# CMUAbstract/VINSat

Measured on AMD Instinct MI355X. Metric: BA iterations/sec (500 poses, 50k landmarks) + final pose RMSE vs ref, higher is better.
Workload: dtype f64; 1 GPU; C3: 500-pose / 50000-observation window, 20-call schedule (10 landmark-only + 10 full); poses=500, observations=50000, windows_per_gpu=1, parallelism=replicas1, devices_visible=1, ranks_per_device=1

## Files before the change

__graft_entry__.py:

```python
import os
import subprocess
import sys

ROOT = os.path.dirname(os.path.abspath(__file__))
if ROOT not in sys.path:
    sys.path.insert(0, ROOT)


def build():
    subprocess.check_call(["make", "-C", os.path.join(ROOT, "vinsat_amd", "csrc"), "-j4"])
    subprocess.call(["make", "-C", os.path.join(ROOT, "tests", "fake_rccl")], stdout=subprocess.DEVNULL, stderr=subprocess.DEVNULL)
    from vinsat_amd import _lib
    lib = _lib.load()
    assert lib.vba_version() >= 100
    import vinsat_amd.ba
    import vinsat_amd.od_pipe


def smoke():
    import numpy as np
    from oracle import ba_oracle as O
    from vinsat_amd import od_pipe, synth
    from vinsat_amd.engine import BAEngine

    lib_path = os.path.join(ROOT, "vinsat_amd", "libvinsat_ba.so")
    if not os.path.exists(lib_path):
        build()
    det, orb = synth.make_sequence("C1")
    win = od_pipe.prepare_window(det, orb)
    st = od_pipe.initial_guess(win)
    n, m = st.shape[0], win.ii.shape[0]
    eng = BAEngine(n, m)
    eng.upload_observations(win.landmarks_xyz, win.landmarks_uv, win.confidences, win.ii, n)
    eng.upload_window(win.intrinsics, win.cumrot_last, win.time_idx)
    lam = 1e-4
    ref, lam_ref = st.copy(), lam
    for it, init in ((0, True), (1, True), (10, False), (11, False)):
        st, lam, hess, ntr, flags = eng.iterate(it, init, lam, st)
        ref, lam_ref, hess_ref, ntr_ref = O.ba_iteration(it, ref, win.cumrot_last, win.landmarks_uv, win.landmarks_xyz,
                                                         win.ii, win.time_idx, win.intrinsics, win.confidences, lam_ref,
                                                         initialize=init)
        err = np.abs(st - ref).max() / np.abs(ref).max()
        assert ntr == ntr_ref and lam == lam_ref, (ntr, ntr_ref, lam, lam_ref)
        assert err < 1e-8, err
    eng.close()
    win2 = od_pipe.prepare_window(*synth.make_two_pass_sequence())
    st2 = win2.states_gt.copy()
    st2[:, :3] += 0.5
    n2, m2 = st2.shape[0], win2.ii.shape[0]
    eng2 = BAEngine(n2, m2)
    eng2.upload_observations(win2.landmarks_xyz, win2.landmarks_uv, win2.confidences, win2.ii, n2)
    eng2.upload_window(win2.intrinsics, win2.cumrot_last, win2.time_idx)
    out2, lam2, _, ntr2, _ = eng2.iterate(12, False, 1e-3, st2)
    ref2, lam_ref2, _, ntr_ref2 = O.ba_iteration(12, st2, win2.cumrot_last, win2.landmarks_uv, win2.landmarks_xyz, win2.ii, win2.time_idx,
                                                win2.intrinsics, win2.confidences, 1e-3, initialize=False)
    err2 = np.abs(out2 - ref2).max() / np.abs(ref2).max()
    assert ntr2 == ntr_ref2 and lam2 == lam_ref2 and err2 < 1e-8, (ntr2, ntr_ref2, lam2, lam_ref2, err2)
    eng2.close()
    print(f"smoke ok: 4 BA calls on cuda:0, max rel state error vs oracle {err:.2e}; a call across gaps of 935 / 510 s {err2:.2e}")


if __name__ == "__main__":
    build()
    if len(sys.argv) > 1 and sys.argv[1] == "smoke":
        smoke()
```

vinsat_amd/csrc/vba_obs.hip:

```cpp
#include "vba_decide.h"
#include <cstdlib>
#include "vba_device.h"
#include "vba_dyn_body.h"
#include "vba_launch.h"
#include "vba_step.h"

namespace vba {

__device__ __forceinline__ void begin_call_scalars(WinScalars& sc, int par, bool keep_wmax = false) {
    sc.done = 0;
    sc.n_trials = 0;
    sc.fl[par] = 0u;
    if (!keep_wmax) sc.wmax_bits[par] = 0ull;
    sc.sum_abs_rpred = 0.0;
}

template <bool HIST0>
__global__ __launch_bounds__(kObsBlock) void k_obs_residual(DevView V, double* abs_out ) {
    __shared__ double red[kObsBlock / 64];
    __shared__ unsigned lh[HIST0 ? 1024 : 1];
    const int w = blockIdx.y;
    VBA_SKIP_CALL(V, w);
    const int m = V.m[w];
    const size_t ob = (size_t)w * V.obs_stride;
// ... 199 lines not shown
    if (blockIdx.x == 0 && threadIdx.x == 0) front_commit(V, w, hit, bin_out, rank_out, in_bin_out, inline_select);
    return hit ? kWarmHit : kWarmMiss;
}

template <int ITEMS>
__global__ __launch_bounds__(256) void k_select_warm(DevView V) {
    __shared__ unsigned lds_u[260];
    __shared__ double red[5][4];
    const int w = blockIdx.y;
    WinScalars& sc = V.sc[w];
    const int t = threadIdx.x;
    const bool fold_here = V.call >= 0 && V.fold && sc.pending == V.call - 1 && sc.call_idx == V.call - 1;
    if (!fold_here) VBA_SKIP_CALL(V, w);
    const double* keys = V.absr + 2 * (size_t)w * V.m_max;
    const int64_t count = 2 * (int64_t)V.m[w];
    if ((int64_t)blockIdx.x * 256 * ITEMS >= count) return;
    constexpr bool PRELOAD = ITEMS <= 8;
    constexpr int PAIRS = ITEMS / 2;
    const double2* keys2 = reinterpret_cast<const double2*>(keys);
    const int64_t npair = count / 2;
    double2 pk[PAIRS];
#pragma unroll
    for (int it = 0; it < PAIRS; ++it) {
        const int64_t idx = ((int64_t)blockIdx.x * PAIRS + it) * 256 + t;
        pk[it] = idx < npair ? keys2[idx] : make_double2(0.0, 0.0);
    }
    const unsigned long long lo = sc.warm_lo[V.par];
    unsigned bin, in_bin;
    long long rank;
    if (warm_front(V, w, fold_here, false, 2 * V.m_max, red, lds_u, bin, rank, in_bin) != kWarmHit) return;
    if constexpr (!PRELOAD) {
        double2 (&kk)[PAIRS] = pk;
        unsigned long long mbits = 0ull;
#pragma unroll
        for (int it = 0; it < PAIRS; ++it) {
            const int64_t idx = ((int64_t)blockIdx.x * PAIRS + it) * 256 + t;
            const bool have = idx < npair;
            if (have && warm_bin(f64_bits(kk[it].x), lo, V.warm_shift) == bin) mbits |= 1ull << (2 * it);
            if (have && warm_bin(f64_bits(kk[it].y), lo, V.warm_shift) == bin) mbits |= 2ull << (2 * it);
        }
        const unsigned mine = (unsigned)__popcll(mbits);
        const unsigned inc = wave_inclusive_scan_u32(mine);
        __syncthreads();
        if ((t & 63) == 63) lds_u[t >> 6] = inc;
        __syncthreads();
        if (t == 0) {
            const unsigned total = lds_u[0] + lds_u[1] + lds_u[2] + lds_u[3];
            lds_u[4] = total ? atomicAdd(&sc.sel_cnt, total) : 0u;
        }
        __syncthreads();
        unsigned at = lds_u[4] + inc - mine;
        for (int q = 0; q < (t >> 6); ++q) at += lds_u[q];
        double* list = V.ckeys + 2 * (size_t)w * V.m_max;
#pragma unroll
        for (int it = 0; it < PAIRS; ++it) {
            if (mbits & (1ull << (2 * it))) list[at++] = kk[it].x;
            if (mbits & (2ull << (2 * it))) list[at++] = kk[it].y;
        }
        return;
    }
    auto take = [&](unsigned long long key, bool have) {
        const bool match = have && warm_bin(key, lo, V.warm_shift) == bin;
        const unsigned long long mask = __ballot(match);
        if (mask) {
            const int lane = t & 63;
            const int leader = __ffsll((long long)mask) - 1;
            unsigned base = 0;
            if (lane == leader) base = atomicAdd(&sc.sel_cnt, (unsigned)__popcll(mask));
            base = (unsigned)__builtin_amdgcn_readlane((int)base, leader);
            if (match) V.ckeys[2 * (size_t)w * V.m_max + base + (unsigned)__popcll(mask & ((1ull << lane) - 1ull))] = bits_f64(key);
        }
    };
    if constexpr (PRELOAD) {
#pragma unroll 8
        for (int it = 0; it < PAIRS; ++it) {
            const int64_t idx = ((int64_t)blockIdx.x * PAIRS + it) * 256 + t;
            const bool have = idx < npair;
            take(f64_bits(pk[it].x), have);
            take(f64_bits(pk[it].y), have);
        }
    }
}

__device__ __forceinline__ double select_finish_list(const DevView& V, int w, const double* ck, int64_t cap, unsigned cnt, long long want,
                                                     int mode, unsigned long long warm_base, bool speculate, unsigned* lh ,
                                                     unsigned* lds_u , unsigned long long* skeys ) {
    const WinScalars& sc = V.sc[w];
    unsigned long long pre[4];
    if (V.sel_nslots > 0 && ck == V.sel_slots) {
        unsigned lo_q = 0;
#pragma unroll
        for (int j = 0; j < 4; ++j) pre[j] = 0ull;
        for (int r = 0; r < V.sel_nslots; ++r) {
            const double* slot = ck + (size_t)r * V.sel_slot_stride;
            const unsigned c_r = (unsigned)slot[0];
#pragma unroll
            for (int j = 0; j < 4; ++j) {
                const unsigned q = threadIdx.x + 256u * j;
                if (q >= lo_q && q < lo_q + c_r && q < cnt) pre[j] = f64_bits(slot[1 + (q - lo_q)]);
            }
            lo_q += c_r;
        }
    } else {
#pragma unroll
        for (int j = 0; j < 4; ++j) {
            const unsigned q = threadIdx.x + 256u * j;
            pre[j] = ((int64_t)q < cap && (speculate || q < cnt)) ? f64_bits(ck[q]) : 0ull;
        }
    }
    if (mode == 1 && cnt <= 1024u && V.warm_shift >= 8) {
        const int t = threadIdx.x;
        const int sh = V.warm_shift - 8;
        lh[t] = 0u;
        if (t == 0) { lds_u[16] = 0u; lds_u[17] = 0u; lds_u[18] = 0u; }
        __syncthreads();
        unsigned sb4[4];
#pragma unroll
        for (int j = 0; j < 4; ++j) {
            const unsigned q = t + 256u * j;
            sb4[j] = (unsigned)((pre[j] - warm_base) >> sh) & 255u;
            if (q < cnt) atomicAdd(&lh[sb4[j]], 1u);
        }
        __syncthreads();
        const unsigned c = lh[t];
        const unsigned inc = wave_inclusive_scan_u32(c);
        if ((t & 63) == 63) lds_u[t >> 6] = inc;
        __syncthreads();
        unsigned base = 0;
        for (int q = 0; q < (t >> 6); ++q) base += lds_u[q];
        const long long excl = (long long)base + inc - c;
        if (want >= excl && want < excl + (long long)c) { lds_u[16] = (unsigned)t; lds_u[17] = (unsigned)(want - excl); }
        __syncthreads();
        const unsigned tb = lds_u[16], r = lds_u[17];
#pragma unroll
        for (int j = 0; j < 4; ++j) {
            const unsigned q = t + 256u * j;
            if (q < cnt && sb4[j] == tb) {
                const unsigned slot = atomicAdd(&lds_u[18], 1u);
                skeys[slot] = pre[j];
            }
        }
        __syncthreads();
        const unsigned k = lds_u[18];
        for (unsigned q = t; q < k; q += 256) {
            const unsigned long long key = skeys[q];
            unsigned below = 0;
            for (unsigned j = 0; j < k; ++j) {
                const unsigned long long o = skeys[j];
                below += (o < key) || (o == key && j < q);
            }
            if (below == r) skeys[1024] = key;
        }
        __syncthreads();
        return bits_f64(skeys[1024]);
    }
    if (cnt <= (mode ? (unsigned)kWarmCount : 1024u)) {
#pragma unroll
        for (int j = 0; j < 4; ++j) {
            const unsigned q = threadIdx.x + 256u * j;
            if (q < cnt) skeys[q] = pre[j];
        }
        __syncthreads();
        for (unsigned q = threadIdx.x; q < cnt; q += 256) {
            const unsigned long long key = skeys[q];
            long long below = 0;
            for (unsigned j = 0; j < cnt; ++j) {
                const unsigned long long o = skeys[j];
                below += (o < key) || (o == key && j < q);
            }
            if (below == want) skeys[1024] = key;
        }
        __syncthreads();
        return bits_f64(skeys[1024]);
    }
    if (mode == 1) {
        unsigned long long prefix = 0ull;
        long long rank = want;
        int remaining = V.warm_shift;
        if (remaining > 11) {
            remaining -= 11;
            for (int b = threadIdx.x; b < kSelBins; b += 256) lh[b] = 0u;
            if (threadIdx.x == 0) lds_u[18] = 0u;
            __syncthreads();
            for (unsigned q = threadIdx.x; q < cnt; q += 256) {
                const unsigned long long rel = f64_bits(ck[q]) - warm_base;
                atomicAdd(&lh[(unsigned)(rel >> remaining) & 2047u], 1u);
            }
            __syncthreads();
            unsigned sub_cnt;
            {
                unsigned loc[8];
                select_load(lh, kSelBins, loc);
// ... 165 lines not shown
            DecideOut d;
            if (!fold_decide(V, w, dec_red, d)) return;
        }
        dynamics_block(V, w, blockIdx.x - nb_acc);
        return;
    }
    const int n = V.n[w];
    if (blockIdx.x * PPB >= n) return;
    VBA_ASTAMP(0);
    const StepParams& prm = V.prm;
    const int sub = threadIdx.x % G;
    const size_t ob = (size_t)w * V.obs_stride;
    const size_t mb = (size_t)w * V.m_max;
    double wmax_l = 0.0;
    const int gstride = BATCH ? (int)gridDim.x : 0;
    int pf_beg = 0, pf_end = 0;
    if (BATCH) {
        const int i0 = blockIdx.x * PPB + threadIdx.x / G;
        if (i0 < n) {
            const int* ptr0 = V.pose_ptr + 2 * ob;
            pf_beg = ptr0[i0];
            pf_end = ptr0[i0 + 1];
        }
    }
    for (int grp = blockIdx.x; grp * PPB < n; grp += gstride) {
    const int i = grp * PPB + threadIdx.x / G;
    const size_t pb = (size_t)w * V.n_max + (i < n ? i : 0);

    struct Obs { double x, y, z, u, v, c; };
    struct alignas(8) D2 { double a, b; };
    struct Obs2 { D2 x, y, z, u, v, c; };
    auto load = [&](int k) {
        Obs o;
        o.x = V.ox[ob + k]; o.y = V.oy[ob + k]; o.z = V.oz[ob + k];
        o.u = V.ou[ob + k]; o.v = V.ov[ob + k]; o.c = V.oconf[ob + k];
        return o;
    };
    auto load2 = [&](int k) {
        Obs2 o;
        o.x = *reinterpret_cast<const D2*>(V.ox + ob + k); o.y = *reinterpret_cast<const D2*>(V.oy + ob + k);
        o.z = *reinterpret_cast<const D2*>(V.oz + ob + k); o.u = *reinterpret_cast<const D2*>(V.ou + ob + k);
        o.v = *reinterpret_cast<const D2*>(V.ov + ob + k); o.c = *reinterpret_cast<const D2*>(V.oconf + ob + k);
        return o;
    };

    unsigned hloc[8] = {};
    if (V.sel_inline && !ordered) select_load(hist0_of(V, w, V.par), kSelBins, hloc);
    PoseCam pc{};
    int beg = 0, end = 0;
    Obs ring[kAccDepth]{};
    Obs2 nxt{}, nxt2{};
#ifndef VBA_ACC_PAIR_DEPTH
#define VBA_ACC_PAIR_DEPTH 1
#endif
    constexpr bool kPairDepth2 = BATCH && PAIR && VBA_ACC_PAIR_DEPTH == 2;
    if (i < n) {
        pose_camera(V.states + pb * 10, V.intr + pb * 4, pc);
        if (BATCH) {
            beg = pf_beg;
            end = pf_end;
        } else {
            beg = early_beg;
            end = early_end;
        }
        if (PAIR) {
            if (beg + 2 * sub < end) nxt = load2(beg + 2 * sub);
            if (kPairDepth2 && beg + 2 * sub + 2 * G < end) nxt2 = load2(beg + 2 * sub + 2 * G);
        } else {
#pragma unroll
            for (int d = 0; d < kAccDepth; ++d)
                if (beg + sub + d * G < end) ring[d] = load(beg + sub + d * G);
        }
    }
    if (BATCH) {
        const int in = i + gstride * PPB;
        pf_beg = pf_end = 0;
        if (in < n) {
            const int* ptr = V.pose_ptr + 2 * ob;
            pf_beg = ptr[in];
            pf_end = ptr[in + 1];
        }
    }

    VBA_ASTAMP(1);
    RobustParams rp;
    if (BATCH) {
        rp.c = sc.c_obs;
    } else if (V.sel_inline) {
        unsigned bin, in_bin;
        long long rank;
        if (ordered) {
            if (warm_front(V, w, fold_here, true, V.bucket_cap, dec_red, sel_u, bin, rank, in_bin) != kWarmHit) return;
        } else {
            if (!front_resolve(V, w, hloc, V.bucket_cap, sel_u, bin, rank, in_bin)) return;
        }
        const unsigned long long lo = sc.warm_lo[V.par];
        const double* bucket = V.wbucket + (((size_t)w * 2 + V.par) * kSelBins + bin) * (size_t)V.bucket_cap;
        rp.c = select_finish_list(V, w, bucket, V.bucket_cap, in_bin, rank, 1, lo + ((unsigned long long)(bin - 1u) << V.warm_shift), false,
                                  sel_lh, sel_u, sel_keys);
        if (ordered && blockIdx.x == 0 && threadIdx.x == 0) sc.c_obs = rp.c;
    } else if (V.median_ready) {
        rp.c = sc.c_obs;
    } else {
        rp.c = select_finish(V, w, sel_lh, sel_u, sel_keys);
        if (blockIdx.x == 0) {
            if (threadIdx.x == 0) sc.c_obs = rp.c;
            unsigned* h0 = hist0_of(V, w, V.par);
            for (int b = threadIdx.x; b < kSelBins; b += 256) h0[b] = 0u;
        }
    }
    VBA_ASTAMP(2);
    rp.inv_c = 1.0 / rp.c;
    rp.inv_c2 = 1.0 / (rp.c * rp.c);
    rp.am2 = prm.am2;
    rp.inv_am2 = 1.0 / prm.am2;
    rp.expo = prm.expo;
    rp.alpha_is_2 = prm.alpha_is_2;
    rp.expo_is_mhalf = prm.expo == -0.5;

    constexpr bool CAM = G <= 16 || F32;
    double acc[32];
#pragma unroll
    for (int q = 0; q < 32; ++q) acc[q] = 0.0;
    double cM[5] = {0, 0, 0, 0, 0}, cT[9] = {0, 0, 0, 0, 0, 0, 0, 0, 0}, cS[3] = {0, 0, 0};
    if (i < n) {
        auto process = [&](double ox_, double oy_, double oz_, double ou_, double ov_, double oc_, int k) {
            double u, v, cam[3], d;
            project(pc, ox_, oy_, oz_, u, v, cam, d);
            const double ru = ou_ - u, rv = ov_ - v;
            const double wr = robust_weight_raw(rp, ru, rv);
            V.wraw[mb + k] = wr;
            wmax_l = fmax(wmax_l, wr);
            const double wc = wr * oc_;
            auto cam_sums = [&](double a00, double a02, double a11, double a12, double g0, double g1, double g2, double h0, double h1,
                                double h2) {
                const double w00 = wc * a00, w02 = wc * a02, w11 = wc * a11, w12 = wc * a12;
                cM[0] = fma(w00, a00, cM[0]); cM[1] = fma(w00, a02, cM[1]);
                cM[2] = fma(w11, a11, cM[2]); cM[3] = fma(w11, a12, cM[3]);
                cM[4] = fma(w02, a02, fma(w12, a12, cM[4]));
                cT[0] = fma(w00, g0, cT[0]); cT[1] = fma(w00, g1, cT[1]); cT[2] = fma(w00, g2, cT[2]);
                cT[3] = fma(w11, h0, cT[3]); cT[4] = fma(w11, h1, cT[4]); cT[5] = fma(w11, h2, cT[5]);
                cT[6] = fma(w02, g0, fma(w12, h0, cT[6])); cT[7] = fma(w02, g1, fma(w12, h1, cT[7]));
                cT[8] = fma(w02, g2, fma(w12, h2, cT[8]));
                const double wg0 = wc * g0, wg1 = wc * g1, wg2 = wc * g2, wh0 = wc * h0, wh1 = wc * h1, wh2 = wc * h2;
                acc[15] = fma(wg0, g0, fma(wh0, h0, acc[15])); acc[16] = fma(wg0, g1, fma(wh0, h1, acc[16]));
                acc[17] = fma(wg0, g2, fma(wh0, h2, acc[17])); acc[18] = fma(wg1, g1, fma(wh1, h1, acc[18]));
                acc[19] = fma(wg1, g2, fma(wh1, h2, acc[19])); acc[20] = fma(wg2, g2, fma(wh2, h2, acc[20]));
                cS[0] = fma(w00, ru, cS[0]); cS[1] = fma(w11, rv, cS[1]); cS[2] = fma(w02, ru, fma(w12, rv, cS[2]));
                acc[24] = fma(wg0, ru, fma(wh0, rv, acc[24])); acc[25] = fma(wg1, ru, fma(wh1, rv, acc[25]));
                acc[26] = fma(wg2, ru, fma(wh2, rv, acc[26]));
            };
            if constexpr (F32) {
                const CamJac32 j = cam_jacobian_f32(pc, cam, d);
                cam_sums(j.a00, j.a02, j.a11, j.a12, j.g0, j.g1, j.g2, j.h0, j.h1, j.h2);
            } else if (CAM) {
                const double live = cam[2] > kZMin ? 1.0 : 0.0;
                const double a00 = pc.fx * d, a11 = pc.fy * d;
                const double dl = d * live;
                const double a02 = -(a00 * (cam[0] * dl)), a12 = -(a11 * (cam[1] * dl));
                const double x = cam[0], y = cam[1], z = cam[2];
                const double b00 = 2.0 * a00, b02 = 2.0 * a02, b11 = 2.0 * a11, b12 = 2.0 * a12;
                const double g0 = -(b02 * y), g1 = fma(b02, x, -(b00 * z)), g2 = b00 * y;
                const double h0 = fma(b11, z, -(b12 * y)), h1 = b12 * x, h2 = -(b11 * x);
                cam_sums(a00, a02, a11, a12, g0, g1, g2, h0, h1, h2);
            } else {
                double J[12];
                project_jacobian(pc, cam, d, J);
                int q = 0;
#pragma unroll
                for (int a = 0; a < 6; ++a) {
                    const double ja = wc * J[a], jb = wc * J[6 + a];
#pragma unroll
                    for (int b = a; b < 6; ++b) { acc[q] = fma(ja, J[b], fma(jb, J[6 + b], acc[q])); ++q; }
                    acc[21 + a] = fma(ja, ru, fma(jb, rv, acc[21 + a]));
                }
            }
        };
        if (PAIR) {
            int k = beg + 2 * sub;
            while (k < end) {
                const int kn = k + 2 * G;
                const Obs2 cur = nxt;
                if (kPairDepth2) {
                    nxt = nxt2;
                    if (kn + 2 * G < end) nxt2 = load2(kn + 2 * G);
                } else if (kn < end) nxt = load2(kn);
                process(cur.x.a, cur.y.a, cur.z.a, cur.u.a, cur.v.a, cur.c.a, k);
                if (k + 1 < end) process(cur.x.b, cur.y.b, cur.z.b, cur.u.b, cur.v.b, cur.c.b, k + 1);
                k = kn;
            }
        } else {
            int k = beg + sub;
            while (k < end) {
                const int kn = k + G;
                const Obs cur = ring[0];
#pragma unroll
                for (int d = 0; d + 1 < kAccDepth; ++d) ring[d] = ring[d + 1];
                if (k + kAccDepth * G < end) ring[kAccDepth - 1] = load(k + kAccDepth * G);
                process(cur.x, cur.y, cur.z, cur.u, cur.v, cur.c, k);
                k = kn;
            }
        }
    }
    VBA_ASTAMP(3);
    if (CAM) {
        const double* R = pc.R;
        const double M[3][3] = {{cM[0], 0.0, cM[1]}, {0.0, cM[2], cM[3]}, {cM[1], cM[3], cM[4]}};
        double Y[3][3];
#pragma unroll
        for (int a = 0; a < 3; ++a)
#pragma unroll
            for (int kk = 0; kk < 3; ++kk) Y[a][kk] = fma(R[3 * a], M[0][kk], fma(R[3 * a + 1], M[1][kk], R[3 * a + 2] * M[2][kk]));
#pragma unroll
        for (int a = 0; a < 3; ++a) {
#pragma unroll
            for (int b = a; b < 3; ++b)
                acc[sym6(a, b)] = fma(Y[a][0], R[3 * b], fma(Y[a][1], R[3 * b + 1], Y[a][2] * R[3 * b + 2]));
#pragma unroll
            for (int c = 0; c < 3; ++c)
                acc[sym6(a, 3 + c)] = -fma(R[3 * a], cT[c], fma(R[3 * a + 1], cT[3 + c], R[3 * a + 2] * cT[6 + c]));
            acc[21 + a] = -fma(R[3 * a], cS[0], fma(R[3 * a + 1], cS[1], R[3 * a + 2] * cS[2]));
        }
    }
    VBA_ASTAMP(4);
    int own = 0;
    halving_steps<G, 32, 1>(acc, sub, own);
    if (G == 64) acc[0] += shfl_xor_f64_c<32>(acc[0]);
    if (i < n && sub < 32) {
        double* H = V.Hraw + pb * 21;
        double* B = V.braw + pb * 6;
        constexpr int kOwn = 32 / (G < 32 ? G : 32);
#pragma unroll
        for (int j = 0; j < kOwn; ++j) {
            const int q = own + j;
            if (q < 21) H[q] = acc[j];
            else if (q < 27) B[q - 21] = acc[j];
        }
    }
    VBA_ASTAMP(5);
    if (!BATCH) break;
    }
    wmax_l = wave_max(wmax_l);
    if ((threadIdx.x & 63) == 0) wmx[threadIdx.x >> 6] = wmax_l;
    __syncthreads();
    if (threadIdx.x == 0) {
        const double mx = fmax(fmax(wmx[0], wmx[1]), fmax(wmx[2], wmx[3]));
        atomicMax(V.wmax_ext ? V.wmax_ext : &sc.wmax_bits[V.par], f64_bits(mx));
    }
    VBA_ASTAMP(6);
}

constexpr int kEdgesPerBlock16 = 15;

template <int EMIT, int FUSED, int PART = 0, int TILES = 1>
__global__ __launch_bounds__(kObsBlock) void k_trial(DevView V) {
    static_assert(PART == 0 || FUSED == 0, "split launches exist for the plain geometry only");
    static_assert(TILES == 1 || (PART == 0 && FUSED == 0), "tiled observation blocks exist for the plain one-grid geometry only");
    constexpr bool FORM = FUSED == 1 || FUSED == 2;
    __shared__ double red[kObsBlock / 64];
    __shared__ double redt[TILES > 1 ? 2 * TILES * (kObsBlock / 64) : 1];
    __shared__ unsigned lh[EMIT == 2 ? kSelBins : (EMIT == 1 ? 1024 : 1)];
    __shared__ double snew[FORM ? (kObsBlock + 1) * 10 : 1];
    __shared__ int lpose[FORM ? kObsBlock : 1];
    __shared__ unsigned wlead[FORM ? 4 : 1];
    const int w = blockIdx.y;
    int early_pose = 0, early_prev = 0;
    constexpr bool kEarlyPose = FUSED == 1 || FUSED == 2;
    if (kEarlyPose && PART != 2) {
        const int64_t ke = min((int64_t)blockIdx.x * kObsBlock + threadIdx.x, V.m_max - 1);
        const int* op = V.opose + 2 * (size_t)w * V.obs_stride;
        early_pose = op[ke];
        early_prev = op[ke > 0 ? ke - 1 : 0];
    }
    VBA_SKIP_CALL(V, w);
    WinScalars& sc = V.sc[w];
// ... 559 lines not shown
```

vinsat_amd/csrc/vba_solve_cr.hip:

```cpp
#include "vba_solve_cr_body.h"

namespace vba {

#ifdef VBA_RESIDENT_STAMPS
VBA_KSTAMP_FETCH(fetch_kstamps_cr)
#endif

template <bool PIVOT>
__global__ __launch_bounds__(256) void k_cr_level01(DevView V, int s) {
    __shared__ __attribute__((aligned(16))) double blk[7 * 252];
    cr_level01_body<PIVOT>(V, s, blockIdx.y, blockIdx.x, blk);
}

template <bool PIVOT>
static void launch_cr_level01_t(const DevView& V, int n0_max, hipStream_t s) {
    hipLaunchKernelGGL(k_cr_level01<PIVOT>, dim3((n0_max + 3) / 4, V.W), dim3(256), 0, s, V, V.chunk);
}
template <bool PIVOT, int PRE>
static void launch_reduced_cr_t(const DevView& V, size_t lds, hipStream_t s) {
    hipLaunchKernelGGL((k_solve_reduced_cr<PIVOT, PRE>), dim3(V.W), dim3(kCrThreads), lds, s, V, V.chunk);
}

static int n0_max_of(const DevView& V) { return (V.n_max + V.chunk - 1) / V.chunk - 1; }
static int n0_min_of(const DevView& V) { return (V.n_min + V.chunk - 1) / V.chunk - 1; }

void launch_cr_tail2(const DevView& V, bool pivot, hipStream_t s) {
    const size_t lds = cr_tail2_lds_bytes(n0_max_of(V));
    if (pivot) launch_reduced_cr_t<true, 2>(V, lds, s);
    else launch_reduced_cr_t<false, 2>(V, lds, s);
}

void launch_cr_front2(const DevView& V, bool pivot, hipStream_t s) {
    const int n0_max = n0_max_of(V);
    if (n0_max < kCrSplitMin) return;
    if (pivot) launch_cr_level01_t<true>(V, n0_max, s);
    else launch_cr_level01_t<false>(V, n0_max, s);
    launch_cr_tail2(V, pivot, s);
}

void launch_cr_short(const DevView& V, bool pivot, hipStream_t s) {
    const int n0_max = n0_max_of(V);
    if (n0_min_of(V) >= kCrSplitMin || n0_max <= 0) return;
    const int nb = n0_max < kCrSplitMin ? n0_max : kCrSplitMin - 1;
    const size_t lds = (size_t)nb * 252 * sizeof(double);
    if (pivot) launch_reduced_cr_t<true, 0>(V, lds, s);
    else launch_reduced_cr_t<false, 0>(V, lds, s);
}

void launch_solve_cr(const DevView& V, bool pivot, hipStream_t s) {
    launch_cr_front2(V, pivot, s);
    launch_cr_short(V, pivot, s);
}

hipError_t configure_cr_device() {
    const LdsLimit set[] = {
        {reinterpret_cast<const void*>(k_solve_reduced_cr<false, 0>), kCrLdsCap}, {reinterpret_cast<const void*>(k_solve_reduced_cr<true, 0>), kCrLdsCap},
        {reinterpret_cast<const void*>(k_solve_reduced_cr<false, 2>), kCrTail2LdsCap}, {reinterpret_cast<const void*>(k_solve_reduced_cr<true, 2>), kCrTail2LdsCap}};
    return set_lds_limits(set);
}

}
```

vinsat_amd/csrc/vba_solve_cr_body.h:

```cpp
#pragma once

#include "vba_solve_step.h"
#include "vba_solve_units.h"

namespace vba {


struct CrLanes {
    int grp, own, ownst;
    int lr, lk;
    int offA[5], offB0[5], offB1[5];
    bool hiB[5];
};

__device__ __forceinline__ CrLanes cr_lanes(int lane) {
    CrLanes g;
    g.grp = lane < 9 ? 0 : (lane < 18 ? 1 : (lane < 27 ? 2 : (lane == 27 ? 3 : 4)));
    const int c = g.grp < 3 ? lane - 9 * g.grp : 0;
    g.own = g.grp == 0 ? 81 + c : (g.grp == 1 ? c : (g.grp == 2 ? 162 + c : 243));
    g.ownst = g.grp == 3 ? 1 : 9;
    g.lr = lane & 15;
    g.lk = lane >> 4;
#pragma unroll
    for (int st = 0; st < 5; ++st) {
// ... 139 lines not shown
        const double* l = cL + (size_t)(in ? q : 0) * 171;
        const double* r_ = cR + (size_t)(in ? q : 0) * 171;
#pragma unroll
        for (int it = 0; it < 2; ++it) {
            const int r = it ? r1 : r0, cc = it ? c1 : c0;
            const bool ok = in && lane + 64 * it < 81;
            lv[u][it] = ok ? l[r * 19 + 1 + cc] : 0.0;
            lw[u][it] = ok ? l[r * 19 + 10 + cc] : 0.0;
            rv[u][it] = ok ? r_[r * 19 + 1 + cc] : 0.0;
            rw[u][it] = ok ? r_[r * 19 + 10 + cc] : 0.0;
            dv[u][it] = ok ? bands[j * 243 + 81 + lane + 64 * it] : 0.0;
        }
        gv[u] = (in && lane < 9) ? rhs[j * 9 + lane] - l[lane * 19] - r_[lane * 19] : 0.0;
    }
    between();
#pragma unroll
    for (int u = 0; u < NB; ++u) {
        const int q = q0 + u * stride;
        if (q >= 0 && q < n1) {
            double* B = dst + (size_t)u * dst_stride * 252;
#pragma unroll
            for (int it = 0; it < 2; ++it) {
                const int i = lane + 64 * it;
                if (i < 81) {
                    const int r = it ? r1 : r0, cc = it ? c1 : c0;
                    B[i] = q == 0 ? 0.0 : -lv[u][it];
                    B[81 + i] = dv[u][it] - lw[u][it] - rv[u][it] + (r == cc ? lam32 : 0.0);
                    B[162 + i] = q == n1 - 1 ? 0.0 : -rw[u][it];
                }
            }
            if (lane < 9) B[243 + lane] = gv[u];
        }
    }
}

template <bool PIVOT>
__device__ __forceinline__ void cr_level01_body(const DevView& V, int s, int w, int t, double* blk) {
    VBA_SKIP_CALL(V, w);
    WinScalars& sc = V.sc[w];
    if (sc.done || !solver_mine<PIVOT>(V, sc)) return;
    const int n1 = n_separators(V.n[w], s);
    if (n1 < kCrSplitMin || n1 > 4 * kCrMax || 4 * t >= n1) return;
    const int lane = threadIdx.x & 63, wv = threadIdx.x >> 6;
    const size_t rb = (size_t)w * V.p_max;
    const double lam32 = (double)(float)sc.lam[V.par];
    const int q0 = 4 * t;
    CrLanes g;
    cr_fill<2>(V, w, s, n1, lam32, q0 + wv, 4, blk + (size_t)wv * 252, 4, lane, [&]() { g = cr_lanes(lane); });
    __syncthreads();
    bool bad = false;
    auto store_P = [&](int u) {
        double* P = V.csol2 + (rb + q0 + u) * 171;
        const double* B = blk + (size_t)u * 252;
        for (int e = lane; e < 171; e += 64) P[e] = e < 81 ? B[e] : B[81 + e];
    };
    if (q0 + 2 * wv < n1) cr_eliminate<PIVOT>(blk + (size_t)(2 * wv) * 252, g, lane, bad);
    __syncthreads();
    if (wv < 3) {
        const int u = 2 * wv + 1;
        if (q0 + u < n1) cr_fold(blk + (size_t)u * 252, blk + (size_t)(u - 1) * 252, blk + (size_t)(u + 1) * 252, q0 + u + 1 < n1, g);
    } else {
        store_P(0);
        if (q0 + 2 < n1) store_P(2);
    }
    __syncthreads();
    if (wv < 2) {
        const int u = 4 * wv + 1;
        if (q0 + u < n1) cr_eliminate<PIVOT>(blk + (size_t)u * 252, g, lane, bad);
    }
    __syncthreads();
    if (wv == 0) {
        if (q0 + 3 < n1) {
            cr_fold(blk + 3 * 252, blk + 1 * 252, blk + 5 * 252, q0 + 5 < n1, g);
            wave_sync_lds();
            double* R = V.cL2 + rb * 171 + (size_t)t * 252;
            for (int e = lane; e < 252; e += 64) R[e] = blk[3 * 252 + e];
        }
    } else if (wv == 1) {
        if (q0 + 1 < n1) store_P(1);
    }
    report_pivot<PIVOT>(bad, sc, lane, V.par);
}

template <bool PIVOT, int PRE, int kCrThreads>
__device__ __forceinline__ void reduced_cr_body(const DevView& V, int s, int w, double* smem) {
    VBA_SKIP_CALL(V, w);
    int tsi = 0;
    const bool tson = threadIdx.x == 0;
    VBA_KSTAMP(tson, tsi++);
    WinScalars& sc = V.sc[w];
    if (sc.done || !solver_mine<PIVOT>(V, sc)) return;
    const int n0 = n_separators(V.n[w], s);
    if (n0 <= 0) return;
    if (PRE ? (n0 < kCrSplitMin || n0 > (PRE == 3 ? 8 : (PRE == 2 ? 4 : 2)) * kCrMax) : (n0 >= kCrSplitMin || n0 > kCrMax)) return;
    const int n1 = PRE == 3 ? n0 / 8 : (PRE == 2 ? n0 / 4 : (PRE ? n0 / 2 : n0));
    const int tid = threadIdx.x, lane = tid & 63, wave = tid >> 6;
    constexpr int NW = kCrThreads / 64;
    const size_t rb = (size_t)w * V.p_max;
    const double lam32 = (double)(float)sc.lam[V.par];
    CrLanes g;
    if (PRE) {
        const double* R = V.cL2 + rb * 171;
        constexpr int kFill = (kCrMax * 252 + kCrThreads - 1) / kCrThreads;
        double v[kFill];
#pragma unroll
        for (int k = 0; k < kFill; ++k) {
            const int idx = tid + k * kCrThreads;
            v[k] = idx < n1 * 252 ? R[idx] : 0.0;
        }
        g = cr_lanes(lane);
#pragma unroll
        for (int k = 0; k < kFill; ++k) {
            const int idx = tid + k * kCrThreads;
            if (idx < n1 * 252) smem[idx] = v[k];
        }
    } else {
        cr_fill<kCrMax / NW>(V, w, s, n1, lam32, wave, NW, smem + (size_t)wave * 252, NW, lane, [&]() { g = cr_lanes(lane); });
    }
    __syncthreads();
    VBA_KSTAMP(tson, tsi++);
    bool bad = false;
    int h = 1, lv = 0;
    for (;; h <<= 1, ++lv) {
        const int cnt = n1 >> lv;
        const int nel = (cnt + 1) / 2;
#pragma nounroll
        for (int t = wave; t < nel; t += NW)
            cr_eliminate<PIVOT>(smem + (size_t)((2 * t + 1) * h - 1) * 252, g, lane, bad);
        __syncthreads();
        VBA_KSTAMP(tson, tsi++);
        if (cnt <= 1) break;
        const int nk = cnt / 2;
#pragma nounroll
        for (int t = wave; t < nk; t += NW) {
            const int j = (2 * t + 2) * h - 1;
            const bool has_p = j + h < n1;
            cr_fold(smem + (size_t)j * 252, smem + (size_t)(j - h) * 252, smem + (size_t)(has_p ? j + h : j) * 252, has_p, g);
        }
        VBA_KSTAMP(tson, 64 + tsi);
        __syncthreads();
        VBA_KSTAMP(tson, tsi++);
    }
    for (; h >= 1; h >>= 1, --lv) {
        const int cnt = n1 >> lv;
        const int nel = (cnt + 1) / 2;
        for (int idx = tid; idx < nel * 9; idx += kCrThreads) {
            const int t = idx / 9, r = idx % 9;
            const int k = (2 * t + 1) * h - 1;
            double* B = smem + (size_t)k * 252;
            double x = B[243 + r];
            if (k - h >= 0) {
                const double* xm = smem + (size_t)(k - h) * 252 + 243;
#pragma unroll
                for (int q = 0; q < 9; ++q) x -= B[r * 9 + q] * xm[q];
            }
            if (k + h < n1) {
                const double* xp = smem + (size_t)(k + h) * 252 + 243;
#pragma unroll
                for (int q = 0; q < 9; ++q) x -= B[162 + r * 9 + q] * xp[q];
            }
            B[243 + r] = x;
        }
        __syncthreads();
        VBA_KSTAMP(tson, tsi++);
    }
    if (PRE == 3) {
        double* x2 = smem + (size_t)n1 * 252;
        double* x1 = x2 + (size_t)((n0 + 7) / 8) * 9;
        auto x_odd = [&](int q) -> const double* {
            return (q & 7) == 7 ? smem + (size_t)(q >> 3) * 252 + 243 : ((q & 7) == 3 ? x2 + (size_t)(q >> 3) * 9 : x1 + (size_t)(q >> 2) * 9);
        };
        auto solve_from = [&](int q, int r, int h) {
            const double* P = V.csol2 + (rb + q) * 171;
            double x = P[162 + r];
            if (q - h >= 0) {
                const double* xm = x_odd(q - h);
#pragma unroll
                for (int k = 0; k < 9; ++k) x -= P[r * 9 + k] * xm[k];
            }
            if (q + h < n0) {
                const double* xp = x_odd(q + h);
#pragma unroll
                for (int k = 0; k < 9; ++k) x -= P[81 + r * 9 + k] * xp[k];
            }
            return x;
        };
        for (int idx = tid; idx < ((n0 + 7) / 8) * 9; idx += kCrThreads) {
            const int q = 8 * (idx / 9) + 3, r = idx % 9;
            if (q < n0) x2[(size_t)(q >> 3) * 9 + r] = solve_from(q, r, 4);
        }
        __syncthreads();
        for (int idx = tid; idx < ((n0 + 3) / 4) * 9; idx += kCrThreads) {
            const int q = 4 * (idx / 9) + 1, r = idx % 9;
            if (q < n0) x1[(size_t)(q >> 2) * 9 + r] = solve_from(q, r, 2);
        }
        __syncthreads();
        for (int idx = tid; idx < n0 * 9; idx += kCrThreads) {
            const int q = idx / 9, r = idx % 9;
            V.rx[rb * 9 + idx] = (q & 1) ? x_odd(q)[r] : solve_from(q, r, 1);
        }
    } else if (PRE == 2) {
        double* x1 = smem + (size_t)n1 * 252;
        auto x_odd = [&](int q) -> const double* {
            return (q & 3) == 3 ? smem + (size_t)(q >> 2) * 252 + 243 : x1 + (size_t)(q >> 2) * 9;
        };
        for (int idx = tid; idx < ((n0 + 3) / 4) * 9; idx += kCrThreads) {
            const int q = 4 * (idx / 9) + 1, r = idx % 9;
            if (q < n0) {
                const double* P = V.csol2 + (rb + q) * 171;
                double x = P[162 + r];
                if (q >= 3) {
                    const double* xm = smem + (size_t)((q - 2) >> 2) * 252 + 243;
#pragma unroll
                    for (int k = 0; k < 9; ++k) x -= P[r * 9 + k] * xm[k];
                }
                if (q + 2 < n0) {
                    const double* xp = smem + (size_t)((q + 2) >> 2) * 252 + 243;
#pragma unroll
                    for (int k = 0; k < 9; ++k) x -= P[81 + r * 9 + k] * xp[k];
                }
                x1[(size_t)(q >> 2) * 9 + r] = x;
            }
        }
        __syncthreads();
        VBA_KSTAMP(tson, tsi++);
        for (int idx = tid; idx < n0 * 9; idx += kCrThreads) {
            const int q = idx / 9, r = idx % 9;
            double x;
            if (q & 1) {
                x = x_odd(q)[r];
            } else {
                const double* P = V.csol2 + (rb + q) * 171;
                x = P[162 + r];
                if (q >= 1) {
                    const double* xm = x_odd(q - 1);
#pragma unroll
                    for (int k = 0; k < 9; ++k) x -= P[r * 9 + k] * xm[k];
                }
                if (q + 1 < n0) {
                    const double* xp = x_odd(q + 1);
#pragma unroll
                    for (int k = 0; k < 9; ++k) x -= P[81 + r * 9 + k] * xp[k];
                }
            }
            V.rx[rb * 9 + idx] = x;
        }
    } else if (!PRE) {
        for (int idx = tid; idx < n1 * 9; idx += kCrThreads) V.rx[rb * 9 + idx] = smem[(size_t)(idx / 9) * 252 + 243 + idx % 9];
    } else {
        for (int idx = tid; idx < n0 * 9; idx += kCrThreads) {
            const int q = idx / 9, r = idx % 9;
            double x;
            if (q & 1) {
                x = smem[(size_t)(q >> 1) * 252 + 243 + r];
            } else {
                const double* P = V.csol2 + (rb + q) * 171;
                x = P[162 + r];
                if (q >= 1) {
                    const double* xm = smem + (size_t)((q - 1) >> 1) * 252 + 243;
#pragma unroll
                    for (int k = 0; k < 9; ++k) x -= P[r * 9 + k] * xm[k];
                }
                if (q + 1 < n0) {
                    const double* xp = smem + (size_t)((q + 1) >> 1) * 252 + 243;
#pragma unroll
                    for (int k = 0; k < 9; ++k) x -= P[81 + r * 9 + k] * xp[k];
                }
            }
            V.rx[rb * 9 + idx] = x;
        }
    }
    VBA_KSTAMP(tson, tsi++);
    (void)tsi; (void)tson;
    report_pivot<PIVOT>(bad, sc, lane, V.par);
}

template <bool PIVOT, int PRE>
__global__ __launch_bounds__(kCrThreads) void k_solve_reduced_cr(DevView V, int s) {
    extern __shared__ __attribute__((aligned(16))) double smem[];
    reduced_cr_body<PIVOT, PRE, kCrThreads>(V, s, blockIdx.x, smem);
}

constexpr size_t cr_tail2_lds_bytes(int n0) { return ((size_t)(n0 / 4) * 252 + (size_t)((n0 + 3) / 4) * 9) * sizeof(double); }
constexpr int kCrLdsCap = kCrMax * 252 * (int)sizeof(double);
constexpr int kCrTail2LdsCap = kCrLdsCap + 65 * 9 * 8;

}
```

Measured before the change: 23200 BA iterations/s.

## Overlap early row projections with median selection and stage CR tail factors in LDS

In the pose accumulation kernel, the first ring of observations is now projected and their Jacobians computed while the robust-scale median selection finishes, using a callback injected into select_finish_list. The ring is refilled with the next batch so selection latency hides the projection math. Separately, the PRE==2 reduced cyclic-reduction tail gains a staged variant that preloads the csol2 factor rows into LDS together with the reduced blocks, so back-substitution reads shared memory instead of global memory. The build also adds a second make invocation with PLAIN_CHAIN=1. The cost is more registers from holding early row terms and more LDS per workgroup for the staged solve, which can lower occupancy.

```diff
diff --git a/__graft_entry__.py b/__graft_entry__.py
--- a/__graft_entry__.py
+++ b/__graft_entry__.py
@@ -9,6 +9,7 @@
 
 def build():
     subprocess.check_call(["make", "-C", os.path.join(ROOT, "vinsat_amd", "csrc"), "-j4"])
+    subprocess.check_call(["make", "-C", os.path.join(ROOT, "vinsat_amd", "csrc"), "-j4", "PLAIN_CHAIN=1"])
     subprocess.call(["make", "-C", os.path.join(ROOT, "tests", "fake_rccl")], stdout=subprocess.DEVNULL, stderr=subprocess.DEVNULL)
     from vinsat_amd import _lib
     lib = _lib.load()
diff --git a/vinsat_amd/csrc/vba_obs.hip b/vinsat_amd/csrc/vba_obs.hip
--- a/vinsat_amd/csrc/vba_obs.hip
+++ b/vinsat_amd/csrc/vba_obs.hip
@@ -305,9 +305,12 @@
     }
 }
 
+struct NoMeanwhile { __device__ __forceinline__ void operator()() const {} };
+template <class Meanwhile = NoMeanwhile>
 __device__ __forceinline__ double select_finish_list(const DevView& V, int w, const double* ck, int64_t cap, unsigned cnt, long long want,
                                                      int mode, unsigned long long warm_base, bool speculate, unsigned* lh ,
-                                                     unsigned* lds_u , unsigned long long* skeys ) {
+                                                     unsigned* lds_u , unsigned long long* skeys ,
+                                                     Meanwhile&& meanwhile = Meanwhile()) {
     const WinScalars& sc = V.sc[w];
     unsigned long long pre[4];
     if (V.sel_nslots > 0 && ck == V.sel_slots) {
@@ -331,6 +334,7 @@
             pre[j] = ((int64_t)q < cap && (speculate || q < cnt)) ? f64_bits(ck[q]) : 0ull;
         }
     }
+    meanwhile();
     if (mode == 1 && cnt <= 1024u && V.warm_shift >= 8) {
         const int t = threadIdx.x;
         const int sh = V.warm_shift - 8;
@@ -662,6 +666,38 @@
         }
     }
 
+#ifdef VBA_NO_EARLY_ROWS
+    constexpr bool EARLY = false;
+#else
+    constexpr bool EARLY = !BATCH && !PAIR && !(G <= 16 || F32);
+#endif
+    struct RowTerms { double ru, rv, J[12], oc; };
+    auto row_terms = [&](const Obs& o) {
+        RowTerms t;
+        double u, v, cam[3], d;
+        project(pc, o.x, o.y, o.z, u, v, cam, d);
+        t.ru = o.u - u;
+        t.rv = o.v - v;
+        project_jacobian(pc, cam, d, t.J);
+        t.oc = o.c;
+        return t;
+    };
+    RowTerms early[EARLY ? kAccDepth : 1]{};
+    bool early_done = false;
+    auto early_rows = [&]() {
+        if constexpr (EARLY) {
+            early_done = true;
+            if (i < n) {
+#pragma unroll
+                for (int d = 0; d < kAccDepth; ++d)
+                    if (beg + sub + d * G < end) early[d] = row_terms(ring[d]);
+#pragma unroll
+                for (int d = 0; d < kAccDepth; ++d)
+                    if (beg + sub + (kAccDepth + d) * G < end) ring[d] = load(beg + sub + (kAccDepth + d) * G);
+            }
+        }
+    };
+
     VBA_ASTAMP(1);
     RobustParams rp;
     if (BATCH) {
@@ -677,7 +713,7 @@
         const unsigned long long lo = sc.warm_lo[V.par];
         const double* bucket = V.wbucket + (((size_t)w * 2 + V.par) * kSelBins + bin) * (size_t)V.bucket_cap;
         rp.c = select_finish_list(V, w, bucket, V.bucket_cap, in_bin, rank, 1, lo + ((unsigned long long)(bin - 1u) << V.warm_shift), false,
-                                  sel_lh, sel_u, sel_keys);
+                                  sel_lh, sel_u, sel_keys, early_rows);
         if (ordered && blockIdx.x == 0 && threadIdx.x == 0) sc.c_obs = rp.c;
     } else if (V.median_ready) {
         rp.c = sc.c_obs;
@@ -689,6 +725,7 @@
             for (int b = threadIdx.x; b < kSelBins; b += 256) h0[b] = 0u;
         }
     }
+    if (!early_done) early_rows();
     VBA_ASTAMP(2);
     rp.inv_c = 1.0 / rp.c;
     rp.inv_c2 = 1.0 / (rp.c * rp.c);
@@ -704,7 +741,25 @@
     for (int q = 0; q < 32; ++q) acc[q] = 0.0;
     double cM[5] = {0, 0, 0, 0, 0}, cT[9] = {0, 0, 0, 0, 0, 0, 0, 0, 0}, cS[3] = {0, 0, 0};
     if (i < n) {
+        auto row_accumulate = [&](const RowTerms& t, int k) {
+            const double wr = robust_weight_raw(rp, t.ru, t.rv);
+            V.wraw[mb + k] = wr;
+            wmax_l = fmax(wmax_l, wr);
+            const double wc = wr * t.oc;
+            int q = 0;
+#pragma unroll
+            for (int a = 0; a < 6; ++a) {
+                const double ja = wc * t.J[a], jb = wc * t.J[6 + a];
+#pragma unroll
+                for (int b = a; b < 6; ++b) { acc[q] = fma(ja, t.J[b], fma(jb, t.J[6 + b], acc[q])); ++q; }
+                acc[21 + a] = fma(ja, t.ru, fma(jb, t.rv, acc[21 + a]));
+            }
+        };
         auto process = [&](double ox_, double oy_, double oz_, double ou_, double ov_, double oc_, int k) {
+            if constexpr (!CAM) {
+                row_accumulate(row_terms(Obs{ox_, oy_, oz_, ou_, ov_, oc_}), k);
+                return;
+            }
             double u, v, cam[3], d;
             project(pc, ox_, oy_, oz_, u, v, cam, d);
             const double ru = ou_ - u, rv = ov_ - v;
@@ -743,17 +798,6 @@
                 const double g0 = -(b02 * y), g1 = fma(b02, x, -(b00 * z)), g2 = b00 * y;
                 const double h0 = fma(b11, z, -(b12 * y)), h1 = b12 * x, h2 = -(b11 * x);
                 cam_sums(a00, a02, a11, a12, g0, g1, g2, h0, h1, h2);
-            } else {
-                double J[12];
-                project_jacobian(pc, cam, d, J);
-                int q = 0;
-#pragma unroll
-                for (int a = 0; a < 6; ++a) {
-                    const double ja = wc * J[a], jb = wc * J[6 + a];
-#pragma unroll
-                    for (int b = a; b < 6; ++b) { acc[q] = fma(ja, J[b], fma(jb, J[6 + b], acc[q])); ++q; }
-                    acc[21 + a] = fma(ja, ru, fma(jb, rv, acc[21 + a]));
-                }
             }
         };
         if (PAIR) {
@@ -771,6 +815,15 @@
             }
         } else {
             int k = beg + sub;
+            if constexpr (EARLY) {
+#pragma unroll
+                for (int d = 0; d < kAccDepth; ++d) {
+                    if (k < end) {
+                        row_accumulate(early[d], k);
+                        k += G;
+                    }
+                }
+            }
             while (k < end) {
                 const int kn = k + G;
                 const Obs cur = ring[0];
diff --git a/vinsat_amd/csrc/vba_solve_cr.hip b/vinsat_amd/csrc/vba_solve_cr.hip
--- a/vinsat_amd/csrc/vba_solve_cr.hip
+++ b/vinsat_amd/csrc/vba_solve_cr.hip
@@ -16,15 +16,23 @@
 static void launch_cr_level01_t(const DevView& V, int n0_max, hipStream_t s) {
     hipLaunchKernelGGL(k_cr_level01<PIVOT>, dim3((n0_max + 3) / 4, V.W), dim3(256), 0, s, V, V.chunk);
 }
-template <bool PIVOT, int PRE>
+template <bool PIVOT, int PRE, bool STAGE = false>
 static void launch_reduced_cr_t(const DevView& V, size_t lds, hipStream_t s) {
-    hipLaunchKernelGGL((k_solve_reduced_cr<PIVOT, PRE>), dim3(V.W), dim3(kCrThreads), lds, s, V, V.chunk);
+    hipLaunchKernelGGL((k_solve_reduced_cr<PIVOT, PRE, STAGE>), dim3(V.W), dim3(kCrThreads), lds, s, V, V.chunk);
 }
 
 static int n0_max_of(const DevView& V) { return (V.n_max + V.chunk - 1) / V.chunk - 1; }
 static int n0_min_of(const DevView& V) { return (V.n_min + V.chunk - 1) / V.chunk - 1; }
 
 void launch_cr_tail2(const DevView& V, bool pivot, hipStream_t s) {
+#ifndef VBA_NO_STAGED_TAIL
+    if (n0_max_of(V) <= kCrStageMaxN0) {
+        const size_t lds_staged = cr_tail2_staged_lds_bytes(n0_max_of(V));
+        if (pivot) launch_reduced_cr_t<true, 2, true>(V, lds_staged, s);
+        else launch_reduced_cr_t<false, 2, true>(V, lds_staged, s);
+        return;
+    }
+#endif
     const size_t lds = cr_tail2_lds_bytes(n0_max_of(V));
     if (pivot) launch_reduced_cr_t<true, 2>(V, lds, s);
     else launch_reduced_cr_t<false, 2>(V, lds, s);
@@ -56,6 +64,13 @@
     const LdsLimit set[] = {
         {reinterpret_cast<const void*>(k_solve_reduced_cr<false, 0>), kCrLdsCap}, {reinterpret_cast<const void*>(k_solve_reduced_cr<true, 0>), kCrLdsCap},
         {reinterpret_cast<const void*>(k_solve_reduced_cr<false, 2>), kCrTail2LdsCap}, {reinterpret_cast<const void*>(k_solve_reduced_cr<true, 2>), kCrTail2LdsCap}};
+#ifndef VBA_NO_STAGED_TAIL
+    constexpr int cap_staged = (int)cr_tail2_staged_lds_bytes(kCrStageMaxN0);
+    static_assert(cap_staged <= kLdsWorkgroupBytes);
+    const LdsLimit staged[] = {{reinterpret_cast<const void*>(k_solve_reduced_cr<false, 2, true>), cap_staged},
+                               {reinterpret_cast<const void*>(k_solve_reduced_cr<true, 2, true>), cap_staged}};
+    if (const hipError_t rc = set_lds_limits(staged); rc != hipSuccess) return rc;
+#endif
     return set_lds_limits(set);
 }
 
diff --git a/vinsat_amd/csrc/vba_solve_cr_body.h b/vinsat_amd/csrc/vba_solve_cr_body.h
--- a/vinsat_amd/csrc/vba_solve_cr_body.h
+++ b/vinsat_amd/csrc/vba_solve_cr_body.h
@@ -245,7 +245,23 @@
     report_pivot<PIVOT>(bad, sc, lane, V.par);
 }
 
-template <bool PIVOT, int PRE, int kCrThreads>
+constexpr size_t cr_tail2_lds_bytes(int n0) { return ((size_t)(n0 / 4) * 252 + (size_t)((n0 + 3) / 4) * 9) * sizeof(double); }
+constexpr int cr_stage_rows(int n0) { return n0 - n0 / 4; }
+constexpr int cr_stage_row_of(int q) { return q - (q >> 2); }
+constexpr size_t cr_tail2_staged_lds_bytes(int n0) { return cr_tail2_lds_bytes(n0) + (size_t)cr_stage_rows(n0) * 171 * sizeof(double); }
+constexpr int kLdsWorkgroupBytes = 160 * 1024;
+constexpr int cr_stage_max_n0() {
+    int n0 = 4 * kCrMax;
+    while (cr_tail2_staged_lds_bytes(n0) > (size_t)kLdsWorkgroupBytes) --n0;
+    return n0;
+}
+#ifdef VBA_NO_STAGED_TAIL
+constexpr int kCrStageMaxN0 = 0;
+#else
+constexpr int kCrStageMaxN0 = cr_stage_max_n0();
+#endif
+
+template <bool PIVOT, int PRE, int kCrThreads, bool STAGE = false>
 __device__ __forceinline__ void reduced_cr_body(const DevView& V, int s, int w, double* smem) {
     VBA_SKIP_CALL(V, w);
     int tsi = 0;
@@ -256,6 +272,7 @@
     const int n0 = n_separators(V.n[w], s);
     if (n0 <= 0) return;
     if (PRE ? (n0 < kCrSplitMin || n0 > (PRE == 3 ? 8 : (PRE == 2 ? 4 : 2)) * kCrMax) : (n0 >= kCrSplitMin || n0 > kCrMax)) return;
+    if (STAGE && n0 > kCrStageMaxN0) return;
     const int n1 = PRE == 3 ? n0 / 8 : (PRE == 2 ? n0 / 4 : (PRE ? n0 / 2 : n0));
     const int tid = threadIdx.x, lane = tid & 63, wave = tid >> 6;
     constexpr int NW = kCrThreads / 64;
@@ -264,18 +281,38 @@
     CrLanes g;
     if (PRE) {
         const double* R = V.cL2 + rb * 171;
-        constexpr int kFill = (kCrMax * 252 + kCrThreads - 1) / kCrThreads;
-        double v[kFill];
+        constexpr int kFillBlocks = STAGE ? kCrStageMaxN0 / 4 : kCrMax;
+        constexpr int kFill = (kFillBlocks * 252 + kCrThreads - 1) / kCrThreads;
+        constexpr int kStage = STAGE ? (cr_stage_rows(kCrStageMaxN0) * 171 + kCrThreads - 1) / kCrThreads : 1;
+        double v[kFill], pv[kStage];
 #pragma unroll
         for (int k = 0; k < kFill; ++k) {
             const int idx = tid + k * kCrThreads;
             v[k] = idx < n1 * 252 ? R[idx] : 0.0;
         }
+        const int nstage = STAGE ? cr_stage_rows(n0) * 171 : 0;
+        if constexpr (STAGE) {
+            const double* P = V.csol2 + rb * 171;
+#pragma unroll
+            for (int k = 0; k < kStage; ++k) {
+                const int e = tid + k * kCrThreads;
+                const int row = e / 171;
+                pv[k] = e < nstage ? P[e + (row / 3) * 171] : 0.0;
+            }
+        }
         g = cr_lanes(lane);
 #pragma unroll
         for (int k = 0; k < kFill; ++k) {
             const int idx = tid + k * kCrThreads;
             if (idx < n1 * 252) smem[idx] = v[k];
+        }
+        if constexpr (STAGE) {
+            double* stage = smem + (size_t)n1 * 252 + (size_t)((n0 + 3) / 4) * 9;
+#pragma unroll
+            for (int k = 0; k < kStage; ++k) {
+                const int e = tid + k * kCrThreads;
+                if (e < nstage) stage[e] = pv[k];
+            }
         }
     } else {
         cr_fill<kCrMax / NW>(V, w, s, n1, lam32, wave, NW, smem + (size_t)wave * 252, NW, lane, [&]() { g = cr_lanes(lane); });
@@ -364,13 +401,17 @@
         }
     } else if (PRE == 2) {
         double* x1 = smem + (size_t)n1 * 252;
+        const double* stage = x1 + (size_t)((n0 + 3) / 4) * 9;
+        auto P_of = [&](int q) -> const double* {
+            return STAGE ? stage + (size_t)cr_stage_row_of(q) * 171 : V.csol2 + (rb + q) * 171;
+        };
         auto x_odd = [&](int q) -> const double* {
             return (q & 3) == 3 ? smem + (size_t)(q >> 2) * 252 + 243 : x1 + (size_t)(q >> 2) * 9;
         };
         for (int idx = tid; idx < ((n0 + 3) / 4) * 9; idx += kCrThreads) {
             const int q = 4 * (idx / 9) + 1, r = idx % 9;
             if (q < n0) {
-                const double* P = V.csol2 + (rb + q) * 171;
+                const double* P = P_of(q);
                 double x = P[162 + r];
                 if (q >= 3) {
                     const double* xm = smem + (size_t)((q - 2) >> 2) * 252 + 243;
@@ -393,7 +434,7 @@
             if (q & 1) {
                 x = x_odd(q)[r];
             } else {
-                const double* P = V.csol2 + (rb + q) * 171;
+                const double* P = P_of(q);
                 x = P[162 + r];
                 if (q >= 1) {
                     const double* xm = x_odd(q - 1);
@@ -438,13 +479,12 @@
     report_pivot<PIVOT>(bad, sc, lane, V.par);
 }
 
-template <bool PIVOT, int PRE>
+template <bool PIVOT, int PRE, bool STAGE = false>
 __global__ __launch_bounds__(kCrThreads) void k_solve_reduced_cr(DevView V, int s) {
     extern __shared__ __attribute__((aligned(16))) double smem[];
-    reduced_cr_body<PIVOT, PRE, kCrThreads>(V, s, blockIdx.x, smem);
-}
-
-constexpr size_t cr_tail2_lds_bytes(int n0) { return ((size_t)(n0 / 4) * 252 + (size_t)((n0 + 3) / 4) * 9) * sizeof(double); }
+    reduced_cr_body<PIVOT, PRE, kCrThreads, STAGE>(V, s, blockIdx.x, smem);
+}
+
 constexpr int kCrLdsCap = kCrMax * 252 * (int)sizeof(double);
 constexpr int kCrTail2LdsCap = kCrLdsCap + 65 * 9 * 8;
 
```

Result: no change. 23100 BA iterations/s, median of 2 (-0.4%).
